# wangkepfe/Real-Time-Ray-Tracing

Measured on AMD Instinct MI355X. Metric: Mray/s + ms/frame at 1080p 4spp (1/2/4/8 GPU); LBVH build ms, higher is better.
Workload: dtype f32; 1 GPU; BASELINE config 3: 1920x1080, 4 spp path trace + SVGF denoise + auto-exposure/tone map, per-frame LBVH rebuild; width=1920, height=1080, spp=4

## Files before the change

### real-time-ray-tracing_amd/csrc/debug_math.hip

```cpp
#include <hip/hip_runtime.h>

#include "rtmath_pk.h"
#include "rtx_amd.h"

namespace {
__global__ __launch_bounds__(256) void k_debug_pk(int fn, const float* x, float y, float c, float* outPk,
                                                  float* outScalar, size_t n) {
    const size_t i = (size_t)blockIdx.x * 256 + threadIdx.x;
    if (i >= n) return;
    const size_t j = (i ^ 1) < n ? (i ^ 1) : i;
    const rtpk::F2 v = {x[i], x[j]};
    float pk = 0.0f, sc = 0.0f;
    if (fn == 0) {
        pk = rtpk::pow_pos2(v, y, rtpk::pow_y_odd(y)).x;
        sc = rt_powf(x[i], y);
    } else if (fn == 1) {
        pk = rtpk::expf2(v).x;
        sc = rt_expf(x[i]);
    } else {
        pk = rtpk::div_rcp2(v, y, c).x;
        sc = rt_div_rcp(x[i], y, c);
    }
    outPk[i] = pk;
    outScalar[i] = sc;
}
}

extern "C" int rt_debug_pk_math(int fn, const float* x, float y, float c, float* out_pk, float* out_scalar, size_t n) {
    if (!x || !out_pk || !out_scalar || fn < 0 || fn > 2) return RT_ERR_ARG;
    if (fn == 0 && !(y > 0.0f && y < __builtin_inff())) return RT_ERR_ARG;
    if (n == 0) return RT_OK;
    hipLaunchKernelGGL(k_debug_pk, dim3((unsigned)((n + 255) / 256)), dim3(256), 0, 0, fn, x, y, c, out_pk, out_scalar, n);
    if (hipGetLastError() != hipSuccess || hipDeviceSynchronize() != hipSuccess) return RT_ERR_HIP;
    return RT_OK;
}
```

### real-time-ray-tracing_amd/csrc/pathtrace.hip

```cpp
#include "emitter_kernels.h"
#include "frame_kernels.h"
#include "launch.h"
#include "pt_common.h"
#include "queue_trace.h"
#include "shade.h"

using namespace rtd;

namespace {

constexpr uint32_t kQShadow = kQShadowFlag;
constexpr int kQSampleShift = 1;
constexpr int kQLightShift = 16;
constexpr int kEmLightBit = 0x40000000;

struct RayState {
    F3 orig, dir, pos, normal, fakeNormal, albedo, centerRaydir;
    int matId, matType, lightIdx, objectIdx;
    bool isRayIntoSurface, hitLight, hit, isDiffuse, isHitProcessed, isOccluded, isShadowRay;
    float offset, normalDotRayDir, depth, rayConeWidth, rayConeSpread;
};

struct PathCtx {
    const PathTraceParams& P;
    F3 sunDir;
    const uint32_t* sob;
    BnPixel bp;
    int frameIdx;
    uint32_t rays, visits, tests, diffuse;
    const float* skyTree = nullptr;
    const float* sunTree = nullptr;
};

RT_DEV PathCtx path_ctx(const PathTraceParams& P, const uint32_t* sob, const float* skyTree, const float* sunTree) {
    return PathCtx{P, f3(P.sunDir[0], P.sunDir[1], P.sunDir[2]), sob, BnPixel{0u, 0u}, 0, 0u, 0u, 0u, 0u, skyTree, sunTree};
}

// ... 64 lines not shown
    if (rs.matType == PERFECT_REFLECTION) {
        rs.dir = normalize(rs.dir - rs.normal * dot(rs.dir, rs.normal) * 2.0f);
        rs.orig = rs.pos + rs.offset * rs.normal;
    } else if (rs.matType == FRESNEL_RR) {
        float etaI = 1.0f, etaT = 1.33f;
        if constexpr (kTab) etaT = mat_vec(c.P, rs.matId, 2).w;
        if (!rs.isRayIntoSurface) { const float t = etaI; etaI = etaT; etaT = t; }
        const float eta = etaI / etaT;
        const float ndr = rs.normalDotRayDir;
        const float cosI = -ndr;
        const float sin2I = max1f(0.0f, (float)(1.0 - (double)(cosI * cosI)));
        const float sin2T = eta * eta * sin2I;
        const float cosT = __builtin_sqrtf(max1f(0.0f, (float)(1.0 - (double)sin2T)));
        F3 next;
        float off = rs.offset;
        if (sin2T >= 1.0f) {
            next = rs.dir - rs.normal * ndr * 2.0f;
        } else {
            const float R1 = etaT * cosI, R2 = etaI * cosT, R3 = etaI * cosI, R4 = etaT * cosT;
            const float Rparl = (R1 - R2) / (R1 + R2), Rperp = (R3 - R4) / (R3 + R4);
            const float fres = (Rparl * Rparl + Rperp * Rperp) / 2.0f;
            if (rnd(c, 0, k) < fres) {
                next = rs.dir - rs.normal * ndr * 2.0f;
            } else {
                next = eta * rs.dir + (eta * cosI - cosT) * rs.normal;
                off = -off;
            }
        }
        rs.dir = normalize(next);
        rs.orig = rs.pos + off * rs.normal;
    }
}

RT_DEV void tri_plane(const PathTraceParams& P, F2 uv, float lod, F3 normal, F3 w, F3& alb, F3& nrm, uint32_t setOff = 0u) {
    uv.x *= 0.5f;
    uv.y *= 0.5f;
    const F4 t0 = sample_lod(P.texAlbedo, uv, lod, setOff);
    __builtin_amdgcn_sched_barrier(0);
    alb = f3(rt_powf_div(t0.x, 2.2f), rt_powf_div(t0.y, 2.2f), rt_powf_div(t0.z, 2.2f));
    __builtin_amdgcn_sched_barrier(0);
    const F4 t1 = sample_lod(P.texNormal, uv, lod, setOff);
    const F3 n = f3(t1.x - 0.5f, t1.y - 0.5f, t1.z - 0.5f);
    const F3 u = cross(normal, w);
    const F3 v = cross(normal, u);
    nrm = normalize(u * n.x + v * n.y + normal * n.z);
}

RT_DEV void sample_emitter(const PathTraceParams& P, F3 from, uint32_t count, float q, float r0, float r1, float rSel,
                           F3& dir, float& pdf, int& lightIdx) {
    float prob;
    const uint32_t slot = emitter_select(P.emCdf, count, rSel, prob);
    const uint32_t tri = P.emTris[slot];
    const float4* tp = P.triPos + 4u * tri;
    const float4 a = tp[0], b = tp[1], d = tp[2];
    const float xyz[9] = {a.x, a.y, a.z, b.x, b.y, b.z, d.x, d.y, d.z};
    float cr[3];
    emitter_cross(xyz, cr);
    const float area = emitter_area(cr);
    const float su = __builtin_sqrtf(r0);
    const float u = 1.0f - su, v = r1 * su;
    const F3 v0 = f3(a.x, a.y, a.z);
    const F3 p = v0 + (f3(b.x, b.y, b.z) - v0) * u + (f3(d.x, d.y, d.z) - v0) * v;
    const F3 to = p - from;
    const float dist2 = to.x * to.x + to.y * to.y + to.z * to.z;
    dir = to / __builtin_sqrtf(dist2);
    const float cosL = fabsf(cr[0] * dir.x + cr[1] * dir.y + cr[2] * dir.z) / (2.0f * area);
    pdf = q * prob * dist2 / (area * cosL);
    lightIdx = (int)tri | kEmLightBit;
}

template <bool kMF, bool kTab = false, bool kNee = false>
RT_DEV void diffuse(PathCtx& c, int bounce, RayState& rs, F3& beta) {
// ... 111 lines not shown
    if (isnan3(beta)) beta = f3(0.0f);
    rs.orig = rs.pos + rs.offset * rs.normal;
}

RT_DEV float ray_cone_width(const PathTraceParams& P, int ix, int iy) {
    const F2 pc = {((float)ix + 0.5f) - P.halfRes[0], ((float)iy + 0.5f) - P.halfRes[1]};
    const F2 po = {copysignf(0.5f, pc.x), copysignf(0.5f, pc.y)};
    const F2 un = {(pc.x - po.x) * P.cam.invRes[0] * 2, (pc.y - po.y) * P.cam.invRes[1] * 2};
    const F2 uf = {(pc.x + po.x) * P.cam.invRes[0] * 2, (pc.y + po.y) * P.cam.invRes[1] * 2};
    const F2 pn = {un.x * P.tanHalfFov[0], un.y * P.tanHalfFov[1]};
    const F2 pf = {uf.x * P.tanHalfFov[0], uf.y * P.tanHalfFov[1]};
    const float an = rt_atanf(__builtin_sqrtf(pn.x * pn.x + pn.y * pn.y));
    const float af = rt_atanf(__builtin_sqrtf(pf.x * pf.x + pf.y * pf.y));
    return af - an;
}

RT_DEV void gbuffer_step0(const PathCtx& c, PathVars& v) {
    const RayState& rs = v.rs;
    v.outDepth = rs.depth;
    v.mask = (uint32_t)rs.matId & 0xFFFFu;
    F2 mv = {0.0f, 0.0f};
    if (rs.hit) {
        const PathTraceParams& P = c.P;
        const F3 d = rs.pos - load3(P.hist.pos);
        const F3 q = f3(dot(load3(P.hist.left), d), dot(load3(P.hist.up), d), dot(load3(P.hist.dir), d));
        const F2 s = {q.x / q.z, q.y / q.z};
        const F2 ndc = {s.x / P.tanHalfFov[0], s.y / P.tanHalfFov[1]};
        mv = F2{(0.5f - ndc.x * 0.5f) - v.sampleUv.x, (0.5f - ndc.y * 0.5f) - v.sampleUv.y};
    }
    v.mv = F2{mv.x + 0.5f, mv.y + 0.5f};
}

template <int kDeferFrom, bool kMF, bool kTab = false, bool kNee = false>
RT_DEV int run_path(PathCtx& c, PathVars& v, int k0, const HitInfo* hit, const SceneView& sc, uint2* stk) {
    RayState& rs = v.rs;
    if (hit) apply_hit<kTab, kNee>(c.P, rs, *hit);
#pragma unroll 1
    for (int k = k0; k < 5; ++k) {
        if ((k != k0 || !hit) && needs_trace(rs)) {
            if (k >= kDeferFrom) return k;
            ++c.rays;
            HitInfo h;
            intersect(sc, rs.orig, rs.dir, stk, 256, h);
            c.visits += h.visits;
            c.tests += h.tests;
            apply_hit<kTab, kNee>(c.P, rs, h);
        }
        if (k == 0) gbuffer_step0(c, v);
        if (k == 4) break;
        glossy<kTab>(c, rs, k);
        if (k >= 2) {
            const bool first = k == 2;
            F3 beta = f3(1.0f);
            diffuse<kMF, kTab, kNee>(c, first ? 0 : 1, rs, beta);
            if (first) {
                v.beta1 = beta;
                v.outNormal = rs.fakeNormal;
            } else {
                v.beta0 = beta;
            }
        }
    }
    return 5;
}

template <bool kMF>
RT_DEV int run_shade0_diffuse(PathCtx& c, PathVars& v, const HitInfo& hit) {
    RayState& rs = v.rs;
    apply_hit(c.P, rs, hit);
    gbuffer_step0(c, v);
    F3 beta = f3(1.0f);
    diffuse<kMF>(c, 0, rs, beta);
    v.beta1 = beta;
    v.outNormal = rs.fakeNormal;
    return needs_trace(rs) ? 3 : 5;
}

template <bool kTab = false>
RT_DEV F3 finish(const PathCtx& c, const PathVars& v) {
    const RayState& rs = v.rs;
    F3 L0 = f3(0.0f);
    if (rs.hitLight && !rs.isOccluded && rs.matType == MAT_SKY) L0 = env_light(c.P, c.sunDir, rs.dir);
    if constexpr (kTab) {
        if (rs.hitLight && !rs.isOccluded && rs.matType == EMISSIVE) {
            const float4 m2 = mat_vec(c.P, rs.matId, 2);
            L0 = f3(m2.x, m2.y, m2.z);
        }
    }
    F3 L2 = L0 * v.beta0 * v.beta1;
    if (isnan3(L2)) L2 = f3(0.0f);
    L2 = f3(clampf(L2.x, 0.0f, 10.0f), clampf(L2.y, 0.0f, 10.0f), clampf(L2.z, 0.0f, 10.0f));
    return L2 / rs.albedo;
}

RT_DEV uint2 pack_h4(float a, float b, float c, uint32_t d16) {
    return make_uint2((uint32_t)rt_f2h(a) | ((uint32_t)rt_f2h(b) << 16), (uint32_t)rt_f2h(c) | (d16 << 16));
}

RT_DEV F3 div_spp(const PathTraceParams& P, F3 v) { return P.invSpp != 0.0f ? v * P.invSpp : v / (float)P.spp; }

RT_DEV uint32_t wave_append(bool want, uint32_t* counter) {
    const unsigned long long m = __ballot(want);
    if (m == 0ull) return 0u;
    const int leader = __ffsll((long long)m) - 1;
    uint32_t base = 0u;
    if ((int)__lane_id() == leader) base = atomicAdd(counter, (uint32_t)__popcll(m));
    base = __shfl(base, leader);
// ... 36 lines not shown
template <bool kBits = false>
RT_DEV void add_rays(const PathTraceParams& P, unsigned long long* wgSlots, uint32_t rays) {
    add_rays<kBits>(P, wgSlots, rays, __builtin_amdgcn_readfirstlane((int)threadIdx.x >> 6));
}

RT_DEV void start_sample(PathCtx& c, PathVars& v, int x, int y, float coneSpread, F3 centerDir) {
    RayState& rs = v.rs;
    v.beta0 = f3(1.0f);
    v.beta1 = f3(1.0f);
    rs.hitLight = false;
    rs.lightIdx = kDefaultLightId;
    rs.isHitProcessed = true;
    rs.isOccluded = false;
    rs.isShadowRay = false;
    rs.isDiffuse = false;
    rs.hit = false;
    rs.matType = MAT_SKY;
    rs.matId = 0;
    rs.objectIdx = -1;
    rs.normal = f3(0.0f, -1.0f, 0.0f);
    rs.fakeNormal = f3(0.0f);
    rs.albedo = f3(1.0f);
    rs.rayConeWidth = 0.0f;
    rs.rayConeSpread = coneSpread;
    rs.centerRaydir = centerDir;
    generate_ray_jittered(c.P.cam, x, y, F2{rnd(c, 0, 0), rnd(c, 0, 1)}, F2{rnd(c, 0, 2), rnd(c, 0, 3)}, rs.orig,
                          rs.dir, v.sampleUv);
    v.outDepth = 0.0f;
    v.mask = 0u;
    v.mv = F2{0.0f, 0.0f};
    v.outNormal = f3(0.0f);
}

}

__host__ __device__ inline int cam_sample_waves(uint32_t spp) { return spp >= 4 ? 4 : (spp >= 2 ? 2 : 1); }
inline bool one_round(uint32_t spp) { return spp >= 1 && ((int)spp + cam_sample_waves(spp) - 1) / cam_sample_waves(spp) == 1; }

template <bool kOneRound, bool kStats>
__global__ __launch_bounds__(256, kOneRound ? 6 : 4) void k_pt_camera(PathTraceParams P) {
    constexpr int kCamLds = 10;
    __shared__ uint2 stk[kCamLds * 256];
    __shared__ uint32_t sob[256];
    __shared__ float4 fold[4][64];
    __shared__ uint32_t surf[4][64];
    __shared__ unsigned long long wgRays[4];
    const int tid = threadIdx.x, lane = tid & 63, w = tid >> 6;
    bn_stage_sobol(P.bluenoise, sob, tid, 256);
    __syncthreads();
    const int nSW = cam_sample_waves(P.spp);
    const int sw = w % nSW, g = w / nSW, tilesX = nSW == 4 ? 1 : 2;
    const int BW = 8 * tilesX, BH = nSW == 1 ? 16 : 8;
    const int x = blockIdx.x * BW + (g % tilesX) * 8 + (lane & 7);
    const int yl = blockIdx.y * BH + (g / tilesX) * 8 + (lane >> 3);
    const bool active = x < (int)P.width && yl < (int)P.rows;
    const int y = (int)row_of(P.y0, P.nStrips, P.strip, (uint32_t)yl);
    const uint32_t p = (uint32_t)y * P.width + (uint32_t)x;
    const uint32_t pl = (uint32_t)yl * P.width + (uint32_t)x;
    const size_t plane = (size_t)P.rows * P.width;
    const SceneView sc = scene_of(P);
    PathCtx c = path_ctx(P, sob, nullptr, nullptr);
    if (active) c.bp = bn_pixel(P.bluenoise, x, y);
    const int rounds = kOneRound ? 1 : ((int)P.spp + nSW - 1) / nSW;
    F3 L = f3(0.0f), A = f3(0.0f);
    bool anyHit = false;
    float4 rec = make_float4(0.0f, 0.0f, 0.0f, 0.0f);
    float recErr = 0.0f;
    uint32_t rays = 0, camV = 0, camT = 0, camCull = 0;
#pragma unroll 1
    for (int r = 0; r < rounds; ++r) {
        const int s = r * nSW + sw;
        float4 out = make_float4(0.0f, 0.0f, 0.0f, 0.0f);
        if (active && s < (int)P.spp) {
            c.frameIdx = (int)P.spp * (P.frameNum - 1) + 1 + s;
            F3 org, dir;
            F2 uv;
            generate_ray_jittered(P.cam, x, y, F2{rnd(c, 0, 0), rnd(c, 0, 1)}, F2{rnd(c, 0, 2), rnd(c, 0, 3)}, org,
                                  dir, uv);
            TravState st;
            if (root_surely_missed(sc, org, dir)) {
// ... 107 lines not shown
    c.next = blockIdx.x;
}
RT_DEV uint32_t claim_next(ShadeClaim& c, uint32_t* counters, uint32_t& slot) {
    if (!c.dyn) {
        const uint32_t b = c.next;
        c.next += gridDim.x;
        return b;
    }
    __syncthreads();
    if (threadIdx.x == 0) {
        uint32_t b = c.batches;
        while (c.drained != (1u << kParts) - 1u) {
            int part = c.home;
            while (c.drained & (1u << part)) part = (part + 1) % kParts;
            const uint32_t got = atomicAdd(&counters[part * 16], 1u);
            const uint32_t lo = (uint32_t)part * c.partLen;
            const uint32_t len = lo >= c.batches ? 0u : (c.batches - lo < c.partLen ? c.batches - lo : c.partLen);
            if (got < len) {
                b = lo + got;
                break;
            }
            c.drained |= 1u << part;
        }
        slot = b;
    }
    __syncthreads();
    return slot;
}

template <bool kGlossy, bool kMF, bool kOneRound, bool kTab = false, bool kNee = false>
#ifndef RTX_SHADE_WAVES
#define RTX_SHADE_WAVES 3
#endif
__global__ __launch_bounds__(256, (kGlossy || !kOneRound) ? 2 : RTX_SHADE_WAVES) void k_pt_shade0(PathTraceParams P) {
    __shared__ uint2 stk[kGlossy ? 17 * 256 : 1];
    __shared__ uint32_t sob[256];
    __shared__ float4 foldL[4][64];
    __shared__ float4 foldA[4][64];
    __shared__ unsigned long long wgRays[4];
    __shared__ __align__(16) float sSkyTree[kSkyTreeNodes];
    __shared__ __align__(16) float sSunTree[kSunTreeNodes];
    __shared__ uint32_t wgBatch;
    const int tid = threadIdx.x, lane = tid & 63, w = tid >> 6;
    const int wS = __builtin_amdgcn_readfirstlane(w);
    bn_stage_sobol(P.bluenoise, sob, tid, 256);
    stage_cdf_trees(P, sSkyTree, sSunTree, tid, 256);
    __syncthreads();
    const uint32_t n = P.ws.counters[kCntSurface];
    const int nSW = cam_sample_waves(P.spp), sw = w % nSW, g = w / nSW;
    const uint32_t perWg = 64u * (uint32_t)(4 / nSW);
    const int rounds = kOneRound ? 1 : ((int)P.spp + nSW - 1) / nSW;
    const SceneView sc = scene_of(P);
    const size_t plane = (size_t)P.rows * P.width;
    uint32_t raysWg = 0, shV = 0, shT = 0, shD = 0;
    ShadeClaim claim;
    claim_init(claim, (n + perWg - 1) / perWg, P.ws.shadeClaim != 0);
#pragma unroll 1
    for (uint32_t base; (base = claim_next(claim, P.ws.fetch + 2 * kParts * 16, wgBatch) * perWg) < n;) {
        const uint32_t i = base + (uint32_t)g * 64u + (uint32_t)lane;
        const bool active = i < n;
        const uint32_t pl = active ? P.ws.surface[i] : 0u;
        const int x = (int)(pl % P.width), yl = (int)(pl / P.width);
        const int y = (int)row_of(P.y0, P.nStrips, P.strip, (uint32_t)yl);
        const uint32_t p = (uint32_t)y * P.width + (uint32_t)x;
        PathCtx c = path_ctx(P, sob, sSkyTree, sSunTree);
        float coneSpread = 0.0f;
        F3 centerDir = f3(0.0f);
        if (active) {
            c.bp = bn_pixel(P.bluenoise, x, y);
            coneSpread = ray_cone_width(P, x, y);
            centerDir = center_dir(P.cam, x, y);
        }
        F3 L = f3(0.0f), A = f3(0.0f), L0s = f3(0.0f), A0s = f3(0.0f), N0 = f3(0.0f);
        float D0 = 0.0f;
        F2 M0 = {0.0f, 0.0f};
        uint32_t mask0 = 0u;
        int sd = -1;
#pragma unroll 1
        for (int r = 0; r < rounds; ++r) {
            const int s = r * nSW + sw;
            const bool run = active && s < (int)P.spp;
            PathVars v;
            int kd = 5;
            if (run) {
                c.frameIdx = (int)P.spp * (P.frameNum - 1) + 1 + s;
                start_sample(c, v, x, y, coneSpread, centerDir);
                const size_t q = (size_t)s * plane + pl;
                const float4 hr = P.ws.hit0Rec[q];
                HitInfo h;
                finalize_hit(sc, v.rs.orig, v.rs.dir, hr.x, (int)__float_as_uint(hr.y), hr.z, hr.w, P.ws.hit0Err[q],
                             h);
                static_assert(!kTab || kGlossy, "the table variant is the all-classes kernel's");
                static_assert(!kNee || kTab, "emitters are entries of a custom table");
                if constexpr (kGlossy) kd = run_path<3, kMF, kTab, kNee>(c, v, 0, &h, sc, stk + tid);
                else kd = run_shade0_diffuse<kMF>(c, v, h);
                if (kd < 3) {
                    atomicAdd(&P.ws.counters[kCntError], 1u);
                    kd = 5;
                }
            }
            const uint32_t slot3 = wave_append(kd == 3, &P.ws.counters[kCntQ3]);
            const uint32_t slot4 = wave_append(kd == 4, &P.ws.counters[kCntQ4]);
            float4 outL = make_float4(0.0f, 0.0f, 0.0f, 0.0f), outA = outL;
            if (run) {
                outA = make_float4(v.rs.albedo.x, v.rs.albedo.y, v.rs.albedo.z, 0.0f);
                if (s == 0) {
                    N0 = v.outNormal;
                    D0 = v.outDepth;
                    M0 = v.mv;
                    mask0 = v.mask;
                }
                if (kd < 5) {
                    ++c.rays;
                    enqueue<kNee>(kd == 3 ? P.ws.q3 : P.ws.q4, kd == 3 ? slot3 : slot4, v, p, (uint32_t)s);
                    outL.w = 1.0f;
                } else {
                    const F3 Ls = finish<kTab>(c, v);
                    outL = make_float4(Ls.x, Ls.y, Ls.z, 0.0f);
                }
            }
            foldL[w][lane] = outL;
            foldA[w][lane] = outA;
            __syncthreads();
            if (sw == 0 && active) {
#pragma unroll 1
                for (int k = 0; k < nSW; ++k) {
                    const int sk = r * nSW + k;
                    if (sk >= (int)P.spp) break;
                    const float4 o = foldL[g * nSW + k][lane];
                    const float4 a = foldA[g * nSW + k][lane];
                    A = A + f3(a.x, a.y, a.z);
                    if (sk == 0) A0s = f3(a.x, a.y, a.z);
                    if (o.w != 0.0f) {
                        if (sd < 0) {
                            sd = sk;
                            if (sk > 0) P.ws.pathL[(size_t)pl * P.spp + sk - 1] = make_float4(L.x, L.y, L.z, 0.0f);
                        }
                    } else {
                        const F3 Ls = f3(o.x, o.y, o.z);
// ... 17 lines not shown
            if (N0.x != N0.x || N0.y != N0.y || N0.z != N0.z) N0 = f3(0.0f);
            if (D0 != D0) D0 = 0.0f;
            if (M0.x != M0.x || M0.y != M0.y) M0 = F2{0.0f, 0.0f};
            if (sd >= 0) {
                P.ws.pending[pslot] = pl | ((uint32_t)sd << 26);
                P.colorOut[p] = make_uint2(0u, mask0 << 16);
            } else {
                P.colorOut[p] = pack_h4(L.x, L.y, L.z, mask0);
            }
            P.normalOut[p] = pack_h4(N0.x, N0.y, N0.z, 0u);
            P.albedoOut[p] = pack_h4(A.x, A.y, A.z, 0u);
            P.depthOut[p] = rt_f2h(D0);
            P.motionOut[p] = (uint32_t)rt_f2h(M0.x) | ((uint32_t)rt_f2h(M0.y) << 16);
        }
        if (active && c.rays) {
            if (P.raysOut) atomicAdd(&P.raysOut[p], c.rays);
            if (P.statsOut) atomicAdd(&P.statsOut[p].x, c.rays);
        }
        if (active && P.statsOut) {
            if (c.visits) atomicAdd(&P.statsOut[p].y, c.visits);
            if (c.tests) atomicAdd(&P.statsOut[p].z, c.tests);
            if (c.diffuse) atomicAdd(&P.statsOut[p].w, c.diffuse);
            shV += c.visits;
            shT += c.tests;
            shD += c.diffuse;
        }
        raysWg += c.rays;
    }
    if (P.statsOut) {
        wave_add(shV, &P.ws.counters[kCntVisShade]);
        wave_add(shT, &P.ws.counters[kCntTstShade]);
        wave_add(shD, &P.ws.counters[kCntDiffShade]);
    }
    add_rays(P, wgRays, raysWg, wS);
}

__global__ __launch_bounds__(256) void k_pt_geom_motion(PathTraceParams P) {
    __shared__ uint32_t sob[256];
    const int tid = threadIdx.x;
    bn_stage_sobol(P.bluenoise, sob, tid, 256);
    __syncthreads();
    const uint32_t n = P.ws.counters[kCntSurface];
    const SceneView sc = scene_of(P);
#pragma unroll 1
    for (uint32_t i = blockIdx.x * 256u + (uint32_t)tid; i < n; i += gridDim.x * 256u) {
        const uint32_t pl = P.ws.surface[i];
        const float4 hr = P.ws.hit0Rec[pl];
        const int tri = (int)__float_as_uint(hr.y);
        if (!(hr.x < kRayMax) || tri < 0) continue;
        const int x = (int)(pl % P.width), yl = (int)(pl / P.width);
        const int y = (int)row_of(P.y0, P.nStrips, P.strip, (uint32_t)yl);
        const uint32_t p = (uint32_t)y * P.width + (uint32_t)x;
        PathCtx c = path_ctx(P, sob, nullptr, nullptr);
        c.bp = bn_pixel(P.bluenoise, x, y);
        c.frameIdx = (int)P.spp * (P.frameNum - 1) + 1;
        PathVars v;
        start_sample(c, v, x, y, 0.0f, f3(0.0f));
        HitInfo h;
        finalize_hit(sc, v.rs.orig, v.rs.dir, hr.x, tri, hr.z, hr.w, P.ws.hit0Err[pl], h);
        const F3 d1 = f3_of(P.triDisp[3 * tri]), d2 = f3_of(P.triDisp[3 * tri + 1]), d3 = f3_of(P.triDisp[3 * tri + 2]);
        v.rs.pos = h.pos - (d3 * (1.0f - hr.z - hr.w) + d1 * hr.z + d2 * hr.w);
        v.rs.hit = true;
        v.rs.depth = h.t;
        gbuffer_step0(c, v);
        F2 M = v.mv;
        if (M.x != M.x || M.y != M.y) M = F2{0.0f, 0.0f};
        P.motionOut[p] = (uint32_t)rt_f2h(M.x) | ((uint32_t)rt_f2h(M.y) << 16);
// ... 55 lines not shown

template <bool kTab = false>
RT_DEV void store_path_L(const PathCtx& c, const PathVars& v, uint32_t p, uint32_t s) {
    const PathTraceParams& P = c.P;
    const F3 Ls = finish<kTab>(c, v);
    const uint32_t pl = local_row(P.y0, P.nStrips, p / P.width) * P.width + p % P.width;
    P.ws.pathL[(size_t)pl * P.spp + s] = make_float4(Ls.x, Ls.y, Ls.z, 0.0f);
}

template <bool kTab = false, bool kNee = false>
RT_DEV uint32_t finish_entry(PathCtx& c, const PathVars& v, bool active, int kd, uint32_t p, uint32_t s, uint32_t& rays,
                             uint32_t& rsD) {
    const PathTraceParams& P = c.P;
    const uint32_t slot = wave_append(kd == 4, &P.ws.counters[kCntQ4]);
    if (active) {
        if (kd < 5) {
            ++c.rays;
            enqueue<kNee>(P.ws.q4, slot, v, p, s);
        } else {
            store_path_L<kTab>(c, v, p, s);
        }
        if (P.raysOut && c.rays) atomicAdd(&P.raysOut[p], c.rays);
        if (P.statsOut) {
            if (c.rays) atomicAdd(&P.statsOut[p].x, c.rays);
            if (c.diffuse) atomicAdd(&P.statsOut[p].w, c.diffuse);
            rsD += c.diffuse;
        }
        rays += c.rays;
    }
    return slot;
}

template <int kStep, bool kMF, bool kGlossy, bool kListed, bool kTab = false, bool kNee = false>
RT_DEV void resume_queue(const PathTraceParams& P) {
    static_assert(!kListed || (kStep == 3 && !kGlossy), "the shading list is queue 3's, kept without glossy tables");
    __shared__ uint32_t sob[256];
    __shared__ unsigned long long wgRays[4];
    __shared__ __align__(16) float sSkyTree[kStep == 3 ? kSkyTreeNodes : 4];
    __shared__ __align__(16) float sSunTree[kStep == 3 ? kSunTreeNodes : 4];
    const uint32_t n = P.ws.counters[kListed ? kCntShade3 : kStep == 3 ? kCntQ3 : kCntQ4];
    if (blockIdx.x * 256u >= n) return;
    const int tid = threadIdx.x;
    bn_stage_sobol(P.bluenoise, sob, tid, 256);
    if (kStep == 3) stage_cdf_trees(P, sSkyTree, sSunTree, tid, 256);
    __syncthreads();
    const PtQueue& q = kStep == 3 ? P.ws.q3 : P.ws.q4;
    const float4* hitRec = kStep == 3 ? P.ws.hitRec : P.ws.hitRec4;
    const float* hitErr = kStep == 3 ? P.ws.hitErr : P.ws.hitErr4;
    const SceneView sc = scene_of(P);
    uint32_t rays = 0, rsD = 0;
#pragma unroll 1
    for (uint32_t base = blockIdx.x * 256u; base < n; base += gridDim.x * 256u) {
        const uint32_t li = base + (uint32_t)tid;
        const bool active = li < n;
        PathCtx c = path_ctx(P, sob, sSkyTree, sSunTree);
        PathVars v;
        int kd = 5;
        uint32_t p = 0, s = 0;
        if (active) {
            const uint32_t i = kListed ? P.ws.shade3[li] : li;
            kd = resume_entry<kStep, kMF, kGlossy, kTab, kNee>(c, q, sc, i, hitRec[i], hitErr[i], v, p, s);
        }
        finish_entry<kTab, kNee>(c, v, active, kd, p, s, rays, rsD);
    }
    if (kStep == 3 && P.statsOut) wave_add(rsD, &P.ws.counters[kCntDiffRes3]);
    add_rays(P, wgRays, rays);
}

template <int kStep, bool kMF, bool kGlossy, bool kTab = false, bool kNee = false>
__global__ __launch_bounds__(256, kStep == 3 ? (kGlossy ? 2 : 3) : 4) void k_pt_resume(PathTraceParams P) {
    static_assert(!kTab || kStep == 4 || (kMF && kGlossy), "the table variant is the all-classes kernel's");
    static_assert(!kNee || kTab, "emitters are entries of a custom table");
    resume_queue<kStep, kMF, kGlossy, false, kTab, kNee>(P);
}

template <bool kMF>
__global__ __launch_bounds__(256, 3) void k_pt_resume3_shade(PathTraceParams P) {
    resume_queue<3, kMF, false, true>(P);
}

__global__ __launch_bounds__(256) void k_pt_resume3_lean(PathTraceParams P) {
    const uint32_t n = P.ws.counters[kCntQ3];
    const SceneView sc = scene_of(P);
#pragma unroll 1
    for (uint32_t i = blockIdx.x * 256u + threadIdx.x; i < n; i += gridDim.x * 256u) {
        const float4 hr = P.ws.hitRec[i];
        if (q3_shades(__float_as_uint(P.ws.q3.rayD[i].w), __float_as_uint(hr.y))) continue;
        PathCtx c = path_ctx(P, nullptr, nullptr, nullptr);
        PathVars v;
        uint32_t p = 0, s = 0;
        HitInfo h;
        reload_entry(c, P.ws.q3, sc, i, hr, P.ws.hitErr[i], v, p, s, h);
        apply_hit(P, v.rs, h);
        if (!(v.rs.hitLight || !v.rs.isDiffuse || v.rs.isOccluded)) atomicAdd(&P.ws.counters[kCntError], 1u);
        store_path_L(c, v, p, s);
    }
}

constexpr int kChainRanges = 32;
#ifndef RTX_CHAIN_STATIC
#define RTX_CHAIN_STATIC 0
#endif
constexpr bool kChainStaticFirst = RTX_CHAIN_STATIC != 0;

template <bool kStats>
RT_DEV bool chain_step(const SceneView& sc, const TravRay& r, TravState& s, TravRec& rec, uint2* stk) {
    return trav_step<16, false, kStats>(sc, r, s, rec, stk, 256, nullptr);
}

#ifndef RTX_CHAIN_WAVES
#define RTX_CHAIN_WAVES 3
#endif
template <bool kStats>
__global__ __launch_bounds__(256, RTX_CHAIN_WAVES) void k_pt_chain(PathTraceParams P) {
    __shared__ uint2 stk[17 * 256];
    __shared__ uint32_t sob[256];
    __shared__ uint2 ranges[4][kChainRanges];
    __shared__ uint32_t q4list[4][64];
    __shared__ unsigned long long wgRays[4];
    const int tid = threadIdx.x, lane = tid & 63, w = __builtin_amdgcn_readfirstlane(tid >> 6);
    bn_stage_sobol(P.bluenoise, sob, tid, 256);
    __syncthreads();
    const uint32_t n = P.ws.counters[kCntQ3];
    const SceneView sc = scene_of(P);
    const PtQueue& q = P.ws.q3;
    Fetch f;
    fetch_init(f, n, gridDim.x * 4u, blockIdx.x * 4u + (uint32_t)w, kChainStaticFirst);
    uint32_t rays = 0, rsD = 0;
#pragma unroll 1
    while (true) {
        uint32_t nRanges = 0;
        if (f.resLo < f.resHi) {
            if (lane == 0) ranges[w][0] = make_uint2(f.resLo, f.resHi);
            nRanges = 1;
        }
        queue_trace<kStats, false, false>(
            sc, f, stk + tid, 256,
            [&] {
                if (f.resLo == f.resHi && nRanges < (uint32_t)kChainRanges) {
                    fetch_topup(f, n, P.ws.fetch, lane);
                    if (f.resLo < f.resHi) {
                        if (lane == 0) ranges[w][nRanges] = make_uint2(f.resLo, f.resHi);
                        ++nRanges;
                    }
                }
            },
            [&] { return fetch_drained(f) || nRanges >= (uint32_t)kChainRanges; },
            [&](uint32_t idx, TravRay& r) {
                const float4 o = q.rayO[idx], d = q.rayD[idx];
                trav_setup(sc, f3(o.x, o.y, o.z), f3(d.x, d.y, d.z), r);
                return (__float_as_uint(d.w) & kQShadowFlag) != 0u;
            },
            [&](uint32_t idx, const TravState& s) {
                P.ws.hitRec[idx] = hit_record(s);
                P.ws.hitErr[idx] = s.hitErrT;
                if (P.statsOut) {
                    const uint32_t p = __float_as_uint(q.rayO[idx].w);
                    atomicAdd(&P.statsOut[p].y, s.visits);
                    atomicAdd(&P.statsOut[p].z, s.tests);
                    atomicMax(&P.ws.counters[kCntMaxIter3], s.iters);
                    atomicAdd(&P.ws.counters[kCntVisQ3], s.visits);
                    atomicAdd(&P.ws.counters[kCntTstQ3], s.tests);
                }
            },
            [](bool, bool, uint32_t, const TravState&) {});
        __builtin_amdgcn_fence(__ATOMIC_SEQ_CST, "workgroup");
        PathCtx c = path_ctx(P, sob, P.skyTree, P.sunTree);
        uint32_t ri = 0, nq4 = 0;
#pragma unroll 1
        while (true) {
            const bool more = ri < nRanges;
            const uint2 rg = more ? ranges[w][ri] : make_uint2(0u, 0u);
            if (nq4 > 0u && (!more || nq4 + (rg.y - rg.x) > 64u)) {
                __builtin_amdgcn_fence(__ATOMIC_SEQ_CST, "workgroup");
                bool act = (uint32_t)lane < nq4;
                const uint32_t slot = act ? q4list[w][lane] : 0u;
                TravRay r4;
                TravState s4;
                {
                    const float4 o = P.ws.q4.rayO[slot], d = P.ws.q4.rayD[slot];
                    trav_setup(sc, f3(o.x, o.y, o.z), f3(d.x, d.y, d.z), r4);
                }
                trav_init(s4, sc.root);
                TravRec rec4;
                const bool mine = act;
                if (nq4 < 16u) {
#pragma unroll 1
                    while (act)
                        if (trav_done(chain_step<kStats>(sc, r4, s4, rec4, stk + tid), s4, true)) act = false;
                } else {
#pragma unroll 1
                    while (__ballot(act) != 0ull) {
                        if (trav_lane_steps(act, s4)) {
                            if (trav_done(chain_step<kStats>(sc, r4, s4, rec4, stk + tid), s4, true)) act = false;
                        }
                    }
                }
                if (mine) {
                    PathVars v;
                    uint32_t p = 0, smp = 0;
                    c.rays = 0;
                    (void)resume_entry<4, false, false>(c, P.ws.q4, sc, slot, hit_record(s4), s4.hitErrT, v, p, smp);
                    store_path_L(c, v, p, smp);
// ... 236 lines not shown
```

### real-time-ray-tracing_amd/csrc/rtmath_pk.h

```cpp
#pragma once
#include "rtmath.h"

namespace rtpk {

typedef float F2 __attribute__((ext_vector_type(2)));
typedef int I2 __attribute__((ext_vector_type(2)));
typedef unsigned int U2 __attribute__((ext_vector_type(2)));

__device__ inline F2 fma2(F2 a, F2 b, F2 c) { return __builtin_elementwise_fma(a, b, c); }
__device__ inline F2 splat(float a) { return F2{a, a}; }
__device__ inline F2 sel(bool c0, bool c1, F2 a, F2 b) { return F2{c0 ? a.x : b.x, c1 ? a.y : b.y}; }
__device__ inline U2 bits2(F2 a) { return __builtin_bit_cast(U2, a); }
__device__ inline F2 from_bits2(U2 a) { return __builtin_bit_cast(F2, a); }

__device__ inline F2 exp2_core2(F2 f) {
    F2 p = splat(1.5252733804059840e-05f);
    p = fma2(p, f, splat(1.5403530393381609e-04f));
    p = fma2(p, f, splat(1.3333558146428443e-03f));
    p = fma2(p, f, splat(9.6181291076284772e-03f));
    p = fma2(p, f, splat(5.5504108664821580e-02f));
    p = fma2(p, f, splat(2.4022650695910071e-01f));
    p = fma2(p, f, splat(6.9314718055994531e-01f));
    return fma2(p, f, splat(1.0f));
}

__device__ inline float scale2_one(float p, int n) {
    const bool hi = n > 127, lo = n < -126;
    const int n1 = hi ? n - 1 : lo ? n + 64 : n;
    const float f2 = hi ? 2.0f : lo ? rtm::bits_to_float((uint32_t)(-64 + 127) << 23) : 1.0f;
    return (p * rtm::bits_to_float((uint32_t)(n1 + 127) << 23)) * f2;
}
__device__ inline F2 scale2_2(F2 p, I2 n) {
    const bool h0 = n.x > 127, h1 = n.y > 127, l0 = n.x < -126, l1 = n.y < -126;
    const I2 n1 = I2{h0 ? n.x - 1 : l0 ? n.x + 64 : n.x, h1 ? n.y - 1 : l1 ? n.y + 64 : n.y};
    const float m64 = rtm::bits_to_float((uint32_t)(-64 + 127) << 23);
    const F2 f2 = F2{h0 ? 2.0f : l0 ? m64 : 1.0f, h1 ? 2.0f : l1 ? m64 : 1.0f};
    const U2 e = __builtin_bit_cast(U2, (n1 + 127) << 23);
    return (p * from_bits2(e)) * f2;
}

__device__ inline F2 exp2_pair2(F2 hi, F2 lo) {
    const F2 hc = __builtin_elementwise_min(__builtin_elementwise_max(hi, splat(-160.0f)), splat(136.0f));
    const F2 n = __builtin_elementwise_rint(hc);
    const F2 f = (hc - n) + lo;
    const F2 r = scale2_2(exp2_core2(f), __builtin_convertvector(n, I2));
    const float inf = rtm::bits_to_float(0x7F800000u);
    return F2{hi.x >= 128.0f ? inf : hi.x < -152.0f ? 0.0f : r.x, hi.y >= 128.0f ? inf : hi.y < -152.0f ? 0.0f : r.y};
}

__device__ inline F2 recip_log_den2(F2 d) {
    F2 y = fma2(splat(-0.239016f), d, splat(0.985076f));
    y = fma2(y, fma2(-d, y, splat(1.0f)), y);
    return fma2(y, fma2(-d, y, splat(1.0f)), y);
}

__device__ inline void log2_pair2(F2 x, F2& hi, F2& lo) {
    const U2 b0 = bits2(x);
    const bool s0 = b0.x < 0x00800000u, s1 = b0.y < 0x00800000u;
    const F2 xs = sel(s0, s1, x * splat(8388608.0f), x);
    const U2 b = bits2(xs);
    I2 e = I2{(int)(b.x >> 23) - (s0 ? 150 : 127), (int)(b.y >> 23) - (s1 ? 150 : 127)};
    F2 m = from_bits2((b & 0x007FFFFFu) | 0x3F800000u);
    const bool f0 = m.x > 1.41421354f, f1 = m.y > 1.41421354f;
    m = sel(f0, f1, m * splat(0.5f), m);
    e = e + I2{f0 ? 1 : 0, f1 ? 1 : 0};
    const F2 r = m - splat(1.0f);
    const F2 d = splat(2.0f) + r, dl = r - (d - splat(2.0f));
    const F2 y = recip_log_den2(d);
    const F2 s0v = r * y;
    const F2 s = fma2(fma2(-s0v, d, r), y, s0v);
    const F2 sl = (fma2(-s, d, r) - s * dl) * y;
    const F2 s2 = s * s;
    F2 q = splat(1.0f / 13.0f);
    q = fma2(q, s2, splat(1.0f / 11.0f));
    q = fma2(q, s2, splat(1.0f / 9.0f));
    q = fma2(q, s2, splat(1.0f / 7.0f));
    q = fma2(q, s2, splat(1.0f / 5.0f));
    q = fma2(q, s2, splat(1.0f / 3.0f));
    const F2 lnh = splat(2.0f) * s;
    const F2 lnl = splat(2.0f) * sl + (splat(2.0f) * s) * (s2 * q);
    const F2 Lh = splat(1.44269502162933349609f), Ll = splat(1.9259629911783e-08f);
    const F2 ph = lnh * Lh;
    const F2 pl = fma2(lnh, Lh, -ph) + fma2(lnh, Ll, lnl * Lh);
    const F2 fe = __builtin_convertvector(e, F2);
    const F2 sh = fe + ph;
    const F2 err = (fe - sh) + ph;
    hi = sh;
    lo = err + pl;
    const F2 t = hi + lo;
    lo = lo - (t - hi);
    hi = t;
}

__device__ inline bool pow_pos_ok(float y) { return y > 0.0f && y < rtm::bits_to_float(0x7F800000u); }
__device__ inline bool pow_y_odd(float y) {
    if (!(__builtin_fabsf(y) < 9007199254740992.0f)) return false;
    const double t = (double)(int64_t)y;
    return t == (double)y && (((int64_t)y) & 1) != 0;
}

__device__ inline F2 pow_pos2(F2 x, float y, bool yOdd) {
    F2 lh, ll;
    log2_pair2(x, lh, ll);
    const F2 Y = splat(y);
    const F2 th = Y * lh;
    const F2 tl = fma2(Y, lh, -th) + Y * ll;
    const F2 r = exp2_pair2(th, tl);
    const U2 xb = bits2(x);
    const float z0 = (xb.x == 0x80000000u && yOdd) ? -0.0f : 0.0f, z1 = (xb.y == 0x80000000u && yOdd) ? -0.0f : 0.0f;
    return F2{x.x == 1.0f ? 1.0f : x.x == 0.0f ? z0 : r.x, x.y == 1.0f ? 1.0f : x.y == 0.0f ? z1 : r.y};
}

__device__ inline F2 expf2(F2 x) {
    const F2 n = __builtin_elementwise_rint(x * splat(1.44269502162933349609f));
    F2 r = fma2(-n, splat(0.693145751953125f), x);
    r = fma2(-n, splat(1.428606765330187e-06f), r);
    F2 p = splat(2.4801587301587302e-05f);
    p = fma2(p, r, splat(1.9841269841269841e-04f));
    p = fma2(p, r, splat(1.3888888888888889e-03f));
    p = fma2(p, r, splat(8.3333333333333333e-03f));
    p = fma2(p, r, splat(4.1666666666666667e-02f));
    p = fma2(p, r, splat(1.6666666666666667e-01f));
    p = fma2(p, r, splat(0.5f));
    p = fma2(p, r, splat(1.0f));
    p = fma2(p, r, splat(1.0f));
    const F2 nc = __builtin_elementwise_min(__builtin_elementwise_max(n, splat(-160.0f)), splat(136.0f));
    const F2 s = scale2_2(p, __builtin_convertvector(nc, I2));
    const float inf = rtm::bits_to_float(0x7F800000u);
    return F2{x.x != x.x ? x.x : x.x > 89.0f ? inf : x.x < -104.0f ? 0.0f : s.x,
              x.y != x.y ? x.y : x.y > 89.0f ? inf : x.y < -104.0f ? 0.0f : s.y};
}

__device__ inline F2 inner3_2g(F2 A, F2 b, F2 C, F2 d, F2 E, F2 f) {
    const F2 ef = E * f, efe = fma2(E, f, -ef);
    const F2 cd = C * d, cde = fma2(C, d, -cd);
    const F2 s2 = cd + ef, dl2 = s2 - cd, s2e = (cd - (s2 - dl2)) + (ef - dl2);
// ... 22 lines not shown
```

Baseline: 11900 Mray/s.

## Pack albedo gamma pow, share per-pixel camera setup across sample waves, reload kernargs

Albedo gamma decoding now evaluates two channels at once through a packed-float pow, falling back to scalar pow for non-finite or negative inputs. In the shade0 kernel, cone spread and center direction are computed by different sample waves and exchanged through shared memory, which adds a workgroup barrier per batch. G-buffer work is skipped for non-first samples via a wave-uniform flag. Kernel parameters are re-read from the kernarg segment inside loops to cut scalar register pressure. Debug-math test hooks are added for the new packed functions.

```diff
diff --git a/real-time-ray-tracing_amd/csrc/debug_math.hip b/real-time-ray-tracing_amd/csrc/debug_math.hip
--- a/real-time-ray-tracing_amd/csrc/debug_math.hip
+++ b/real-time-ray-tracing_amd/csrc/debug_math.hip
@@ -9,9 +9,19 @@
     const size_t i = (size_t)blockIdx.x * 256 + threadIdx.x;
     if (i >= n) return;
     const size_t j = (i ^ 1) < n ? (i ^ 1) : i;
-    const rtpk::F2 v = {x[i], x[j]};
+    const bool second = (fn & 0x100) != 0;
+    fn &= 0xFF;
+    const rtpk::F2 v = second ? rtpk::F2{x[j], x[i]} : rtpk::F2{x[i], x[j]};
     float pk = 0.0f, sc = 0.0f;
-    if (fn == 0) {
+    if (fn == 3) {
+        const rtpk::F2 r = rtpk::unorm16_2((uint32_t)v.x, (uint32_t)v.y);
+        pk = second ? r.y : r.x;
+        sc = rt_unorm16((uint32_t)x[i]);
+    } else if (fn == 4) {
+        const rtpk::F2 r = rtpk::pow_pos2<true>(v, y, rtpk::pow_y_odd(y));
+        pk = second ? r.y : r.x;
+        sc = rt_powf_div(x[i], y);
+    } else if (fn == 0) {
         pk = rtpk::pow_pos2(v, y, rtpk::pow_y_odd(y)).x;
         sc = rt_powf(x[i], y);
     } else if (fn == 1) {
@@ -27,8 +37,9 @@
 }
 
 extern "C" int rt_debug_pk_math(int fn, const float* x, float y, float c, float* out_pk, float* out_scalar, size_t n) {
-    if (!x || !out_pk || !out_scalar || fn < 0 || fn > 2) return RT_ERR_ARG;
-    if (fn == 0 && !(y > 0.0f && y < __builtin_inff())) return RT_ERR_ARG;
+    const int f = fn & 0xFF;
+    if (!x || !out_pk || !out_scalar || fn < 0 || f > 4 || (fn & ~0x1FF) != 0 || ((fn & 0x100) != 0 && f < 3)) return RT_ERR_ARG;
+    if ((f == 0 || f == 4) && !(y > 0.0f && y < __builtin_inff())) return RT_ERR_ARG;
     if (n == 0) return RT_OK;
     hipLaunchKernelGGL(k_debug_pk, dim3((unsigned)((n + 255) / 256)), dim3(256), 0, 0, fn, x, y, c, out_pk, out_scalar, n);
     if (hipGetLastError() != hipSuccess || hipDeviceSynchronize() != hipSuccess) return RT_ERR_HIP;
diff --git a/real-time-ray-tracing_amd/csrc/pathtrace.hip b/real-time-ray-tracing_amd/csrc/pathtrace.hip
--- a/real-time-ray-tracing_amd/csrc/pathtrace.hip
+++ b/real-time-ray-tracing_amd/csrc/pathtrace.hip
@@ -3,6 +3,7 @@
 #include "launch.h"
 #include "pt_common.h"
 #include "queue_trace.h"
+#include "rtmath_pk.h"
 #include "shade.h"
 
 using namespace rtd;
@@ -133,12 +134,21 @@
     }
 }
 
+RT_DEV F3 gamma3(float x, float y, float z) {
+    const float inf = rtm::bits_to_float(0x7F800000u);
+    const rtpk::F2 xy = rtpk::pow_pos2<true>(rtpk::F2{x, y}, 2.2f, false);
+    float gx = xy.x, gy = xy.y;
+    if (!(x >= 0.0f && x < inf)) gx = rt_powf_div(x, 2.2f);
+    if (!(y >= 0.0f && y < inf)) gy = rt_powf_div(y, 2.2f);
+    return f3(gx, gy, rt_powf_div(z, 2.2f));
+}
+
 RT_DEV void tri_plane(const PathTraceParams& P, F2 uv, float lod, F3 normal, F3 w, F3& alb, F3& nrm, uint32_t setOff = 0u) {
     uv.x *= 0.5f;
     uv.y *= 0.5f;
     const F4 t0 = sample_lod(P.texAlbedo, uv, lod, setOff);
     __builtin_amdgcn_sched_barrier(0);
-    alb = f3(rt_powf_div(t0.x, 2.2f), rt_powf_div(t0.y, 2.2f), rt_powf_div(t0.z, 2.2f));
+    alb = gamma3(t0.x, t0.y, t0.z);
     __builtin_amdgcn_sched_barrier(0);
     const F4 t1 = sample_lod(P.texNormal, uv, lod, setOff);
     const F3 n = f3(t1.x - 0.5f, t1.y - 0.5f, t1.z - 0.5f);
@@ -316,7 +326,7 @@
 }
 
 template <int kDeferFrom, bool kMF, bool kTab = false, bool kNee = false>
-RT_DEV int run_path(PathCtx& c, PathVars& v, int k0, const HitInfo* hit, const SceneView& sc, uint2* stk) {
+RT_DEV int run_path(PathCtx& c, PathVars& v, int k0, const HitInfo* hit, const SceneView& sc, uint2* stk, bool s0 = true) {
     RayState& rs = v.rs;
     if (hit) apply_hit<kTab, kNee>(c.P, rs, *hit);
 #pragma unroll 1
@@ -330,7 +340,7 @@
             c.tests += h.tests;
             apply_hit<kTab, kNee>(c.P, rs, h);
         }
-        if (k == 0) gbuffer_step0(c, v);
+        if (k == 0 && s0) gbuffer_step0(c, v);
         if (k == 4) break;
         glossy<kTab>(c, rs, k);
         if (k >= 2) {
@@ -339,7 +349,7 @@
             diffuse<kMF, kTab, kNee>(c, first ? 0 : 1, rs, beta);
             if (first) {
                 v.beta1 = beta;
-                v.outNormal = rs.fakeNormal;
+                if (s0) v.outNormal = rs.fakeNormal;
             } else {
                 v.beta0 = beta;
             }
@@ -349,14 +359,14 @@
 }
 
 template <bool kMF>
-RT_DEV int run_shade0_diffuse(PathCtx& c, PathVars& v, const HitInfo& hit) {
+RT_DEV int run_shade0_diffuse(PathCtx& c, PathVars& v, const HitInfo& hit, bool s0) {
     RayState& rs = v.rs;
     apply_hit(c.P, rs, hit);
-    gbuffer_step0(c, v);
+    if (s0) gbuffer_step0(c, v);
     F3 beta = f3(1.0f);
     diffuse<kMF>(c, 0, rs, beta);
     v.beta1 = beta;
-    v.outNormal = rs.fakeNormal;
+    if (s0) v.outNormal = rs.fakeNormal;
     return needs_trace(rs) ? 3 : 5;
 }
 
@@ -459,6 +469,13 @@
     v.outNormal = f3(0.0f);
 }
 
+RT_DEV const PathTraceParams& params_at_use(const PathTraceParams&) {
+    typedef const __attribute__((address_space(4))) PathTraceParams* KernArg;
+    KernArg k = (KernArg)__builtin_amdgcn_kernarg_segment_ptr();
+    asm volatile("" : "+s"(k));
+    return *(const PathTraceParams*)k;
+}
+
 }
 
 __host__ __device__ inline int cam_sample_waves(uint32_t spp) { return spp >= 4 ? 4 : (spp >= 2 ? 2 : 1); }
@@ -472,7 +489,7 @@
     __shared__ float4 fold[4][64];
     __shared__ uint32_t surf[4][64];
     __shared__ unsigned long long wgRays[4];
-    const int tid = threadIdx.x, lane = tid & 63, w = tid >> 6;
+    const int tid = threadIdx.x, lane = tid & 63, w = __builtin_amdgcn_readfirstlane(tid >> 6);
     bn_stage_sobol(P.bluenoise, sob, tid, 256);
     __syncthreads();
     const int nSW = cam_sample_waves(P.spp);
@@ -646,7 +663,8 @@
 #ifndef RTX_SHADE_WAVES
 #define RTX_SHADE_WAVES 3
 #endif
-__global__ __launch_bounds__(256, (kGlossy || !kOneRound) ? 2 : RTX_SHADE_WAVES) void k_pt_shade0(PathTraceParams P) {
+__global__ __launch_bounds__(256, (kGlossy || !kOneRound) ? 2 : RTX_SHADE_WAVES) void k_pt_shade0(PathTraceParams Pk) {
+    const PathTraceParams& P = Pk;
     __shared__ uint2 stk[kGlossy ? 17 * 256 : 1];
     __shared__ uint32_t sob[256];
     __shared__ float4 foldL[4][64];
@@ -655,8 +673,8 @@
     __shared__ __align__(16) float sSkyTree[kSkyTreeNodes];
     __shared__ __align__(16) float sSunTree[kSunTreeNodes];
     __shared__ uint32_t wgBatch;
-    const int tid = threadIdx.x, lane = tid & 63, w = tid >> 6;
-    const int wS = __builtin_amdgcn_readfirstlane(w);
+    __shared__ float4 sPix[2][64];
+    const int tid = threadIdx.x, lane = tid & 63, w = __builtin_amdgcn_readfirstlane(tid >> 6);
     bn_stage_sobol(P.bluenoise, sob, tid, 256);
     stage_cdf_trees(P, sSkyTree, sSunTree, tid, 256);
     __syncthreads();
@@ -664,13 +682,14 @@
     const int nSW = cam_sample_waves(P.spp), sw = w % nSW, g = w / nSW;
     const uint32_t perWg = 64u * (uint32_t)(4 / nSW);
     const int rounds = kOneRound ? 1 : ((int)P.spp + nSW - 1) / nSW;
-    const SceneView sc = scene_of(P);
-    const size_t plane = (size_t)P.rows * P.width;
     uint32_t raysWg = 0, shV = 0, shT = 0, shD = 0;
     ShadeClaim claim;
     claim_init(claim, (n + perWg - 1) / perWg, P.ws.shadeClaim != 0);
 #pragma unroll 1
     for (uint32_t base; (base = claim_next(claim, P.ws.fetch + 2 * kParts * 16, wgBatch) * perWg) < n;) {
+        const PathTraceParams& P = params_at_use(Pk);
+        const SceneView sc = scene_of(P);
+        const size_t plane = (size_t)P.rows * P.width;
         const uint32_t i = base + (uint32_t)g * 64u + (uint32_t)lane;
         const bool active = i < n;
         const uint32_t pl = active ? P.ws.surface[i] : 0u;
@@ -680,10 +699,26 @@
         PathCtx c = path_ctx(P, sob, sSkyTree, sSunTree);
         float coneSpread = 0.0f;
         F3 centerDir = f3(0.0f);
+        const bool shared = nSW > 1;
         if (active) {
             c.bp = bn_pixel(P.bluenoise, x, y);
-            coneSpread = ray_cone_width(P, x, y);
-            centerDir = center_dir(P.cam, x, y);
+            if (!shared || sw == 0) coneSpread = ray_cone_width(P, x, y);
+            if (!shared || sw == 1) centerDir = center_dir(P.cam, x, y);
+        }
+        if (shared) {
+            if (active && sw == 0) sPix[g][lane].w = coneSpread;
+            if (active && sw == 1) {
+                float4& d = sPix[g][lane];
+                d.x = centerDir.x;
+                d.y = centerDir.y;
+                d.z = centerDir.z;
+            }
+            __syncthreads();
+            if (active) {
+                const float4 pv = sPix[g][lane];
+                coneSpread = pv.w;
+                centerDir = f3(pv.x, pv.y, pv.z);
+            }
         }
         F3 L = f3(0.0f), A = f3(0.0f), L0s = f3(0.0f), A0s = f3(0.0f), N0 = f3(0.0f);
         float D0 = 0.0f;
@@ -694,6 +729,7 @@
         for (int r = 0; r < rounds; ++r) {
             const int s = r * nSW + sw;
             const bool run = active && s < (int)P.spp;
+            const bool s0 = __builtin_amdgcn_readfirstlane(s) == 0;
             PathVars v;
             int kd = 5;
             if (run) {
@@ -706,8 +742,8 @@
                              h);
                 static_assert(!kTab || kGlossy, "the table variant is the all-classes kernel's");
                 static_assert(!kNee || kTab, "emitters are entries of a custom table");
-                if constexpr (kGlossy) kd = run_path<3, kMF, kTab, kNee>(c, v, 0, &h, sc, stk + tid);
-                else kd = run_shade0_diffuse<kMF>(c, v, h);
+                if constexpr (kGlossy) kd = run_path<3, kMF, kTab, kNee>(c, v, 0, &h, sc, stk + tid, s0);
+                else kd = run_shade0_diffuse<kMF>(c, v, h, s0);
                 if (kd < 3) {
                     atomicAdd(&P.ws.counters[kCntError], 1u);
                     kd = 5;
@@ -718,7 +754,7 @@
             float4 outL = make_float4(0.0f, 0.0f, 0.0f, 0.0f), outA = outL;
             if (run) {
                 outA = make_float4(v.rs.albedo.x, v.rs.albedo.y, v.rs.albedo.z, 0.0f);
-                if (s == 0) {
+                if (s0) {
                     N0 = v.outNormal;
                     D0 = v.outDepth;
                     M0 = v.mv;
@@ -802,7 +838,7 @@
         wave_add(shT, &P.ws.counters[kCntTstShade]);
         wave_add(shD, &P.ws.counters[kCntDiffShade]);
     }
-    add_rays(P, wgRays, raysWg, wS);
+    add_rays(P, wgRays, raysWg, w);
 }
 
 __global__ __launch_bounds__(256) void k_pt_geom_motion(PathTraceParams P) {
@@ -924,7 +960,8 @@
 }
 
 template <int kStep, bool kMF, bool kGlossy, bool kListed, bool kTab = false, bool kNee = false>
-RT_DEV void resume_queue(const PathTraceParams& P) {
+RT_DEV void resume_queue(const PathTraceParams& Pk) {
+    const PathTraceParams& P = Pk;
     static_assert(!kListed || (kStep == 3 && !kGlossy), "the shading list is queue 3's, kept without glossy tables");
     __shared__ uint32_t sob[256];
     __shared__ unsigned long long wgRays[4];
@@ -936,13 +973,14 @@
     bn_stage_sobol(P.bluenoise, sob, tid, 256);
     if (kStep == 3) stage_cdf_trees(P, sSkyTree, sSunTree, tid, 256);
     __syncthreads();
-    const PtQueue& q = kStep == 3 ? P.ws.q3 : P.ws.q4;
-    const float4* hitRec = kStep == 3 ? P.ws.hitRec : P.ws.hitRec4;
-    const float* hitErr = kStep == 3 ? P.ws.hitErr : P.ws.hitErr4;
-    const SceneView sc = scene_of(P);
     uint32_t rays = 0, rsD = 0;
 #pragma unroll 1
     for (uint32_t base = blockIdx.x * 256u; base < n; base += gridDim.x * 256u) {
+        const PathTraceParams& P = params_at_use(Pk);
+        const PtQueue& q = kStep == 3 ? P.ws.q3 : P.ws.q4;
+        const float4* hitRec = kStep == 3 ? P.ws.hitRec : P.ws.hitRec4;
+        const float* hitErr = kStep == 3 ? P.ws.hitErr : P.ws.hitErr4;
+        const SceneView sc = scene_of(P);
         const uint32_t li = base + (uint32_t)tid;
         const bool active = li < n;
         PathCtx c = path_ctx(P, sob, sSkyTree, sSunTree);
@@ -1004,7 +1042,8 @@
 #define RTX_CHAIN_WAVES 3
 #endif
 template <bool kStats>
-__global__ __launch_bounds__(256, RTX_CHAIN_WAVES) void k_pt_chain(PathTraceParams P) {
+__global__ __launch_bounds__(256, RTX_CHAIN_WAVES) void k_pt_chain(PathTraceParams Pk) {
+    const PathTraceParams& P = Pk;
     __shared__ uint2 stk[17 * 256];
     __shared__ uint32_t sob[256];
     __shared__ uint2 ranges[4][kChainRanges];
@@ -1014,13 +1053,14 @@
     bn_stage_sobol(P.bluenoise, sob, tid, 256);
     __syncthreads();
     const uint32_t n = P.ws.counters[kCntQ3];
-    const SceneView sc = scene_of(P);
-    const PtQueue& q = P.ws.q3;
     Fetch f;
     fetch_init(f, n, gridDim.x * 4u, blockIdx.x * 4u + (uint32_t)w, kChainStaticFirst);
     uint32_t rays = 0, rsD = 0;
 #pragma unroll 1
     while (true) {
+        const PathTraceParams& P = params_at_use(Pk);
+        const SceneView sc = scene_of(P);
+        const PtQueue& q = P.ws.q3;
         uint32_t nRanges = 0;
         if (f.resLo < f.resHi) {
             if (lane == 0) ranges[w][0] = make_uint2(f.resLo, f.resHi);
@@ -1057,10 +1097,13 @@
             },
             [](bool, bool, uint32_t, const TravState&) {});
         __builtin_amdgcn_fence(__ATOMIC_SEQ_CST, "workgroup");
-        PathCtx c = path_ctx(P, sob, P.skyTree, P.sunTree);
         uint32_t ri = 0, nq4 = 0;
 #pragma unroll 1
         while (true) {
+            const PathTraceParams& P = params_at_use(Pk);
+            const SceneView sc = scene_of(P);
+            const PtQueue& q = P.ws.q3;
+            PathCtx c = path_ctx(P, sob, P.skyTree, P.sunTree);
             const bool more = ri < nRanges;
             const uint2 rg = more ? ranges[w][ri] : make_uint2(0u, 0u);
             if (nq4 > 0u && (!more || nq4 + (rg.y - rg.x) > 64u)) {
diff --git a/real-time-ray-tracing_amd/csrc/rtmath_pk.h b/real-time-ray-tracing_amd/csrc/rtmath_pk.h
--- a/real-time-ray-tracing_amd/csrc/rtmath_pk.h
+++ b/real-time-ray-tracing_amd/csrc/rtmath_pk.h
@@ -54,6 +54,13 @@
     return fma2(y, fma2(-d, y, splat(1.0f)), y);
 }
 
+__device__ inline F2 unorm16_2(uint32_t x, uint32_t y) {
+    const F2 xf = F2{(float)x, (float)y}, c = splat(rtm::bits_to_float(0x37800080u));
+    const F2 q = xf * c;
+    return fma2(fma2(-q, splat(65535.0f), xf), c, q);
+}
+
+template <bool kDiv = false>
 __device__ inline void log2_pair2(F2 x, F2& hi, F2& lo) {
     const U2 b0 = bits2(x);
     const bool s0 = b0.x < 0x00800000u, s1 = b0.y < 0x00800000u;
@@ -66,10 +73,17 @@
     e = e + I2{f0 ? 1 : 0, f1 ? 1 : 0};
     const F2 r = m - splat(1.0f);
     const F2 d = splat(2.0f) + r, dl = r - (d - splat(2.0f));
-    const F2 y = recip_log_den2(d);
-    const F2 s0v = r * y;
-    const F2 s = fma2(fma2(-s0v, d, r), y, s0v);
-    const F2 sl = (fma2(-s, d, r) - s * dl) * y;
+    F2 s, sl;
+    if (kDiv) {
+        s = F2{r.x / d.x, r.y / d.y};
+        const F2 num = fma2(-s, d, r) - s * dl;
+        sl = F2{num.x / d.x, num.y / d.y};
+    } else {
+        const F2 y = recip_log_den2(d);
+        const F2 s0v = r * y;
+        s = fma2(fma2(-s0v, d, r), y, s0v);
+        sl = (fma2(-s, d, r) - s * dl) * y;
+    }
     const F2 s2 = s * s;
     F2 q = splat(1.0f / 13.0f);
     q = fma2(q, s2, splat(1.0f / 11.0f));
@@ -99,9 +113,10 @@
     return t == (double)y && (((int64_t)y) & 1) != 0;
 }
 
+template <bool kDiv = false>
 __device__ inline F2 pow_pos2(F2 x, float y, bool yOdd) {
     F2 lh, ll;
-    log2_pair2(x, lh, ll);
+    log2_pair2<kDiv>(x, lh, ll);
     const F2 Y = splat(y);
     const F2 th = Y * lh;
     const F2 tl = fma2(Y, lh, -th) + Y * ll;
```

Result: no change. 11890 Mray/s, median of 2 (-0.1%).
